# stanFurrer/Robust-Multimodal-Contrastive-Learning

Hardware: AMD Instinct MI355X
Metric: image-text pairs/sec, ViLT-B/32 RMCL step (PGD K=3) (higher is better)
Workload: dtype bf16; 1 GPU; RMCL step, PGD K=3 image attack + MoCo InfoNCE (queue 65536) + full backward + AdamW, ViLT-B/32, bs=64/GPU, 384x384 img + 40 tok (BASELINE configs[2]; [3] when n_gpus=8); global_batch=64, parallelism=dp1, grad_sync=ring/f32, ln_fold=on (shift-robust form)

## Files before the change

### robust-multimodal-contrastive-learning_amd/csrc/api.cpp

```cpp
#include "rmcl_common.h"
#include "kernels.h"
#include "../../include/rmcl.h"
#include <mutex>
#include <string>
#include <unordered_set>

static thread_local std::string g_err;
extern "C" void rmcl_set_error(const char* msg) { g_err = msg ? msg : ""; }

int rmcl_attention_fwd_impl(const void* qkv, const int* mask, void* out, void* probs, float* scores, int B, int N, int H, int dt,
                            int exact, hipStream_t s);
int rmcl_attention_bwd_impl(const void* qkv, const int* mask, const void* probs, const void* dout, const void* out, void* dqkv,
                            float* scores, void* dS, int B, int N, int H, int dt, int exact, hipStream_t s);

#include <vector>
namespace {
struct Prof {
  bool on = false;
  int mask = 0;
  size_t n = 0, cap = 0;
  std::vector<hipEvent_t> ev;
  double flops = 0.0;
} g_prof;
}
// ... 59 lines not shown
  g_prof.on = false;
  double ms = 0.0;
  for (size_t i = 0; i < g_prof.n; ++i) {
    hipError_t r = hipEventSynchronize(g_prof.ev[2 * i + 1]);
    float t = 0.f;
    if (r == hipSuccess) r = hipEventElapsedTime(&t, g_prof.ev[2 * i], g_prof.ev[2 * i + 1]);
    if (r != hipSuccess) { rmcl_set_error(hipGetErrorString(r)); return (int)r; }
    ms += t;
  }
  if (ms_total) *ms_total = ms;
  if (launches) *launches = (int64_t)g_prof.n;
  if (flops_total) *flops_total = g_prof.flops;
  return 0;
}
int rmcl_version(void) { return 1; }

int rmcl_dropout_mask_apply(float* x, int64_t n, uint32_t drop_seed, int layer, int site, float drop_p, void* stream) {
  RMCL_REQUIRE(x && drop_p >= 0.f && drop_p < 1.f, "dropout_mask_apply: bad argument");
  if (drop_p == 0.f) return 0;
  return rmcl_dropout_apply(x, n, rmcl_site_seed(drop_seed, layer, site), (uint32_t)((double)drop_p * 4294967296.0), 1.0f / (1.0f - drop_p),
                            (hipStream_t)stream);
}
extern int g_st_reserve_cus;
extern bool g_attn_fused_bwd;
extern bool g_dw_grouped;
extern int g_attn_fwd_waves;
extern int g_infonce_fold;
extern int g_dp_stagger;
extern int g_attn_bwd_persist;
extern int g_attn_bwd_tpw;
extern int g_gemm_share;
extern bool g_lnfold_centred;
extern int g_prefetch_mask, g_prefetch_wgs;
int rmcl_l2_prefetch_experiment(const void* A, int64_t lda_bytes, int M, int rows_per_tile, int tiles_per_xcd, int col_tiles, const void* B,
                                int64_t ldb_bytes, int nB, int nk, int tick, int lead, int per_xcd, int wgs, int* counter, int64_t* stamps, void* stream) {
  RMCL_REQUIRE(A && B && counter && M > 0 && nk > 0 && per_xcd > 0 && wgs > 0 && col_tiles > 0, "l2_prefetch_experiment: bad argument");
  return rmcl_debug_l2_prefetch(A, (long)lda_bytes, M, rows_per_tile, tiles_per_xcd, col_tiles, B, (long)ldb_bytes, nB, nk, tick, lead, per_xcd, wgs, counter,
                                reinterpret_cast<long long*>(stamps), (hipStream_t)stream);
}
int rmcl_tune_set(int key, int value) {
  if (key == 11) { g_lnfold_centred = value != 0; return 0; }
  if (key == 12) { g_prefetch_mask = value & 7; return 0; }
  if (key == 13) { g_prefetch_wgs = value < 0 ? 0 : (value > 64 ? 64 : value); return 0; }
  if (key == 7) { g_dp_stagger = value < 0 ? 0 : value; return 0; }
  if (key == 10) { g_gemm_share = value < 1 ? 1 : (value > 8 ? 8 : value); return 0; }
  if (key == 9) { g_attn_bwd_tpw = value; return 0; }
  if (key == 8) { g_attn_bwd_persist = value < 0 ? 0 : value; return 0; }
  if (key == 6) { rmcl_gemm_skinny_set_form(value); return 0; }
  if (key == 0) { rmcl_gemm_fast_set_cfg(value); return 0; }
  if (key == 1) { g_st_reserve_cus = value < 0 ? 0 : (value > 128 ? 128 : value); return 0; }
  if (key == 2) { g_attn_fused_bwd = value != 0; return 0; }
  if (key == 5) { g_infonce_fold = value != 0; return 0; }
  if (key == 4) { g_attn_fwd_waves = value; return 0; }
  if (key == 3) { g_dw_grouped = value != 0; return 0; }
  rmcl_set_error("tune_set: unknown key");
  return -1;
}

int64_t rmcl_heads_stash_bytes(const rmcl_dims* d) { return (int64_t)carve_heads(*d, nullptr, nullptr) + 256; }

int rmcl_heads_forward(const rmcl_dims* d, const float* pool32, const float* head32, const float* xn, void* hstash,
                       float* cls_feats, float* q, void* stream) {
  return rmcl_heads_forward2(d, pool32, head32, xn, hstash, cls_feats, q, 0, stream);
}
int rmcl_heads_forward2(const rmcl_dims* d, const float* pool32, const float* head32, const float* xn, void* hstash,
                        float* cls_feats, float* q, int flags, void* stream) {
  RMCL_REQUIRE(d && pool32 && xn && hstash && cls_feats, "heads_forward: NULL argument");
  RMCL_REQUIRE((flags & ~RMCL_HEADS_NO_WGRAD) == 0, "heads_forward: unknown flag");
  rmcl_layout y;
  rmcl_param_layout(d, &y);
  HeadStash h;
  carve_heads(*d, hstash, &h);
  hipStream_t s = (hipStream_t)stream;
  const int B = d->B, D = d->D, N = d->L + 1 + d->P;
  const bool stash_in = !(flags & RMCL_HEADS_NO_WGRAD);
  {
// ... 353 lines not shown
```

### robust-multimodal-contrastive-learning_amd/csrc/gemm_st.hip

```cpp
#include "rmcl_common.h"
#include "kernels.h"

#define ST_OP_BYTES (ST_T * 128)
#define ST_STAGE (2 * ST_OP_BYTES)
#define ST_LDS (3 * ST_STAGE)


#ifdef ST_TRACE
#ifndef ST_TRACE_WG
#define ST_TRACE_WG 100
#endif
__device__ long long g_st_trace[2][32];
#define ST_STAMP(i)                                                                                              \
  if (blockIdx.x == ST_TRACE_WG && (threadIdx.x & 255) == 0) g_st_trace[threadIdx.x >> 8][i] = wall_clock64()
extern "C" int rmcl_debug_st_trace(long long* out) {
  return (int)hipMemcpyFromSymbol(out, HIP_SYMBOL(g_st_trace), sizeof(long long) * 64);
}
__device__ long long g_dw_trace[2][32];
#define DW_STAMP(i)                                                                                              \
  if (blockIdx.x == ST_TRACE_WG && (threadIdx.x & 255) == 0) g_dw_trace[threadIdx.x >> 8][i] = wall_clock64()
extern "C" int rmcl_debug_dw_trace(long long* out) {
  return (int)hipMemcpyFromSymbol(out, HIP_SYMBOL(g_dw_trace), sizeof(long long) * 64);
}
#else
// ... 19 lines not shown
__device__ __forceinline__ bf16x8 st_ld_b(const char* lds_b, int off, int s) {
  if (KC) {
    return *reinterpret_cast<const bf16x8*>(lds_b + off);
  } else {
    union { bf16x8 v; s16x4 h[2]; } u;
    const uint32_t a = lds_addr(lds_b + off);
    if (s == 0) { u.h[0] = lds_read_tr16_asm<0>(a); u.h[1] = lds_read_tr16_asm<4 * 384>(a); }
    else { u.h[0] = lds_read_tr16_asm<32 * 384>(a); u.h[1] = lds_read_tr16_asm<32 * 384 + 4 * 384>(a); }
    return u.v;
  }
}

#define ST_PHASE_BEGIN()                                  \
  __builtin_amdgcn_sched_barrier(0);                      \
  __builtin_amdgcn_s_barrier();                           \
  asm volatile("s_waitcnt lgkmcnt(0)" ::: "memory");      \
  __builtin_amdgcn_sched_barrier(0);                      \
  __builtin_amdgcn_s_setprio(1)
#define ST_PHASE_END()                                    \
  __builtin_amdgcn_s_setprio(0);                          \
  __builtin_amdgcn_sched_barrier(0);                      \
  __builtin_amdgcn_s_barrier();                           \
  __builtin_amdgcn_sched_barrier(0)

struct STCtx {
  const bf16_t* A;
  const bf16_t* B;
  uint32_t oa[3], ob[3];
  int aoff[2], aoffi[6], boff[2], boffj[3];
  long kstep_a, kstep_b;
  int wave;
};

template <int MODE, bool A_KC, bool B_KC, int PH>
__device__ __forceinline__ void st_tile(f32x4 (&acc)[6][3], const STCtx& c, const char* cur, char* nxt2, int t2) {
  if constexpr (PH == 2) {
    bf16x8 a[6], b[3];
#pragma unroll
    for (int s = 0; s < 2; ++s) {
#pragma unroll
      for (int j = 0; j < 3; ++j) b[j] = B_KC ? st_ld_b<true>(cur + ST_OP_BYTES, j * 2048 + c.boff[s], s) : st_ld_b<false>(cur + ST_OP_BYTES, c.boffj[j], s);
#pragma unroll
      for (int i = 0; i < 6; ++i) a[i] = A_KC ? st_ld_b<true>(cur, i * 2048 + c.aoff[s], s) : st_ld_b<false>(cur, c.aoffi[i], s);
      if (MODE == 0) {
        if (s == 0) st_stage_op(c.A, c.oa, (long)t2 * c.kstep_a, nxt2, c.wave);
        else { st_stage_op(c.B, c.ob, (long)t2 * c.kstep_b, nxt2 + ST_OP_BYTES, c.wave); st_wait_vm<6>(); }
      } else if (MODE == 1 && s == 1) {
        st_wait_vm<0>();
      }
      asm volatile("s_waitcnt lgkmcnt(0)" ::: "memory");
      ST_PHASE_BEGIN();
#pragma unroll
      for (int i = 0; i < 6; ++i)
#pragma unroll
        for (int j = 0; j < 3; ++j) acc[i][j] = __builtin_amdgcn_mfma_f32_16x16x32_bf16(b[j], a[i], acc[i][j], 0, 0, 0);
      ST_PHASE_END();
    }
  } else {
    bf16x8 a[2][6], b[2][3];
#pragma unroll
    for (int s = 0; s < 2; ++s) {
#pragma unroll
      for (int j = 0; j < 3; ++j) b[s][j] = B_KC ? st_ld_b<true>(cur + ST_OP_BYTES, j * 2048 + c.boff[s], s) : st_ld_b<false>(cur + ST_OP_BYTES, c.boffj[j], s);
#pragma unroll
      for (int i = 0; i < 6; ++i) a[s][i] = A_KC ? st_ld_b<true>(cur, i * 2048 + c.aoff[s], s) : st_ld_b<false>(cur, c.aoffi[i], s);
    }
    if (MODE == 0) {
      st_stage_op(c.A, c.oa, (long)t2 * c.kstep_a, nxt2, c.wave);
      st_stage_op(c.B, c.ob, (long)t2 * c.kstep_b, nxt2 + ST_OP_BYTES, c.wave);
      st_wait_vm<6>();
    } else if (MODE == 1) {
      st_wait_vm<0>();
    }
    asm volatile("s_waitcnt lgkmcnt(0)" ::: "memory");
    ST_PHASE_BEGIN();
#pragma unroll
    for (int s = 0; s < 2; ++s)
#pragma unroll
      for (int i = 0; i < 6; ++i)
// ... 77 lines not shown
      float v[4] = {g.alpha * acc[i][j][0] + bias[j].x, g.alpha * acc[i][j][1] + bias[j].y, g.alpha * acc[i][j][2] + bias[j].z,
                    g.alpha * acc[i][j][3] + bias[j].w};
      if (DROP && (epi & EPI_DROP_BWD)) {
        const uint32_t di = (uint32_t)((long)m * g.ld_aux + nb + j * 16);
        drop_scale4(g.drop_seed, di, g.drop_thresh, g.drop_inv_keep, v[0], v[1], v[2], v[3]);
      }
      if (AUX == ST_AUX_DGELU) {
        const uint2 u = pre[i][j];
        v[0] *= gelu_poly_grad(__uint_as_float(u.x << 16)); v[1] *= gelu_poly_grad(__uint_as_float(u.x & 0xffff0000u));
        v[2] *= gelu_poly_grad(__uint_as_float(u.y << 16)); v[3] *= gelu_poly_grad(__uint_as_float(u.y & 0xffff0000u));
      }
      const long ci = (long)m * g.ldc + nb + j * 16;
      if ((epi & EPI_SAVE_PREACT) && live) st_store4<TO>(C2 + ci, v);
      if (epi & EPI_GELU) {
#pragma unroll
        for (int r = 0; r < 4; ++r) v[r] = gelu_poly(v[r]);
      }
      if (DROP && (epi & EPI_DROPOUT)) {
        drop_scale4(g.drop_seed, (uint32_t)ci, g.drop_thresh, g.drop_inv_keep, v[0], v[1], v[2], v[3]);
      }
      if (AUX == ST_AUX_RES) { v[0] += res[i][j].x; v[1] += res[i][j].y; v[2] += res[i][j].z; v[3] += res[i][j].w; }
      if constexpr (sizeof(TO) == 4) {
        if ((epi & EPI_ACCUM) && live) {
          const float4 o = *reinterpret_cast<const float4*>(C + ci);
          v[0] += o.x; v[1] += o.y; v[2] += o.z; v[3] += o.w;
        }
      }
      if (live) st_store4<TO>(C + ci, v);
    }
  }
}


template <bool A_KC, bool B_KC, int AUX, typename TO, bool DROP, int PH, int LNF = 0>
__global__ __launch_bounds__(512) void gemm_st_kernel(GemmArgs g, int tiles_m, int tiles_n, int rows_per_tile, int xflags) {
  extern __shared__ __attribute__((aligned(16))) char smem[];
  const int t = threadIdx.x, lane = t & 63;
  const int wave = __builtin_amdgcn_readfirstlane(t >> 6);
  const int wm = wave >> 2, wn = wave & 3;
  const int ntiles = tiles_m * tiles_n * max(g.splitk, 1), G = gridDim.x, bidx = blockIdx.x;

  STCtx c;
  c.A = reinterpret_cast<const bf16_t*>(g.A);
  c.B = reinterpret_cast<const bf16_t*>(g.B);
  c.wave = wave;
  c.kstep_a = A_KC ? 64 : 64 * g.lda;
  c.kstep_b = B_KC ? 64 : 64 * g.ldb;
#pragma unroll
  for (int i = 0; i < 6; ++i) {
    const int q = (lane & 15) >> 2, p = lane & 3;
    const int k = 8 * (lane >> 4) + q;
    const int c8 = (wm * 96 + i * 16) / 4 + p;
    c.aoffi[i] = k * 384 + (((c8 >> 1) ^ (st_gk(k) << 1)) * 16) + (c8 & 1) * 8;
  }
#pragma unroll
  for (int s = 0; s < 2; ++s) {
    const int sw = ((4 * s + (lane >> 4)) ^ (lane & 7)) * 16;
    c.aoff[s] = (wm * 96 + (lane & 15)) * 128 + sw;
    c.boff[s] = (wn * 48 + (lane & 15)) * 128 + sw;
  }
#pragma unroll
  for (int j = 0; j < 3; ++j) {
    const int q = (lane & 15) >> 2, p = lane & 3;
    const int k = 8 * (lane >> 4) + q;
    const int c8 = (wn * 48 + j * 16) / 4 + p;
    c.boffj[j] = k * 384 + (((c8 >> 1) ^ (st_gk(k) << 1)) * 16) + (c8 & 1) * 8;
  }

  ST_STAMP(0);
  int id = st_tile_id(bidx, 0, G, ntiles);
  if (id < 0) return;
  STTile cur, nxt;
  st_tile_setup<A_KC, B_KC>(cur, g, id, tiles_m, tiles_n, rows_per_tile, wave, lane, xflags);
#pragma unroll
  for (int q = 0; q < 3; ++q) { c.oa[q] = cur.oa[q]; c.ob[q] = cur.ob[q]; }

  st_stage_op(c.A, c.oa, (long)cur.kt0 * c.kstep_a, smem, wave);
  st_stage_op(c.B, c.ob, (long)cur.kt0 * c.kstep_b, smem + ST_OP_BYTES, wave);
  st_stage_op(c.A, c.oa, (long)(cur.kt0 + 1) * c.kstep_a, smem + ST_STAGE, wave);
  st_stage_op(c.B, c.ob, (long)(cur.kt0 + 1) * c.kstep_b, smem + ST_STAGE + ST_OP_BYTES, wave);
  st_wait_vm<6>();
  __builtin_amdgcn_s_barrier();
  __builtin_amdgcn_sched_barrier(0);
  if (wm == 1) __builtin_amdgcn_s_barrier();
  __builtin_amdgcn_sched_barrier(0);

  ST_STAMP(1);
  int sc = 0, sn = 2;
  for (int r = 0;; ++r) {
    const int nid = st_tile_id(bidx, r + 1, G, ntiles);
    f32x4 acc[6][3];
#pragma unroll
    for (int i = 0; i < 6; ++i)
#pragma unroll
      for (int j = 0; j < 3; ++j) acc[i][j] = f32x4{0.f, 0.f, 0.f, 0.f};
    const int nk = cur.nk;
    for (int it = 0; it + 2 < nk; ++it) {
      st_tile<0, A_KC, B_KC, PH>(acc, c, smem + sc * ST_STAGE, smem + sn * ST_STAGE, cur.kt0 + it + 2);
      sc = sc == 2 ? 0 : sc + 1;
      sn = sn == 2 ? 0 : sn + 1;
    }
    if (nid >= 0) {
      st_tile_setup<A_KC, B_KC>(nxt, g, nid, tiles_m, tiles_n, rows_per_tile, wave, lane, xflags);
#pragma unroll
      for (int q = 0; q < 3; ++q) { c.oa[q] = nxt.oa[q]; c.ob[q] = nxt.ob[q]; }
#pragma unroll
      for (int e = 0; e < 2; ++e) {
        st_tile<0, A_KC, B_KC, PH>(acc, c, smem + sc * ST_STAGE, smem + sn * ST_STAGE, nxt.kt0 + e);
        sc = sc == 2 ? 0 : sc + 1;
        sn = sn == 2 ? 0 : sn + 1;
      }
    } else {
      st_tile<1, A_KC, B_KC, PH>(acc, c, smem + sc * ST_STAGE, nullptr, 0);
      sc = sc == 2 ? 0 : sc + 1;
      st_tile<2, A_KC, B_KC, PH>(acc, c, smem + sc * ST_STAGE, nullptr, 0);
    }
    ST_STAMP(2);
    const int s_free = nid >= 0 ? (sc == 0 ? 2 : sc - 1) : sc;
    st_epilogue_lds<AUX, TO, DROP, LNF>(acc, g, cur, wm, wn, lane, wave, smem + s_free * ST_STAGE + wm * (ST_STAGE / 2),
                                        reinterpret_cast<float*>(smem + ST_LDS));
    if (nid < 0) break;
    cur = nxt;
  }
  ST_STAMP(20);
  if (wm == 0) __builtin_amdgcn_s_barrier();
#ifdef ST_TRACE
  asm volatile("s_waitcnt vmcnt(0)" ::: "memory");
  ST_STAMP(21);
#endif
}

__global__ __launch_bounds__(512) void gemm_dw_group_kernel(DwGroupArgs a) {
  extern __shared__ __attribute__((aligned(16))) char smem[];
  const int t = threadIdx.x, lane = t & 63;
  const int wave = __builtin_amdgcn_readfirstlane(t >> 6);
  const int wm = wave >> 2, wn = wave & 3;
  DW_STAMP(0);
  if ((int)blockIdx.x < a.nslots * ((a.D + 255) / 256) && t < 256) {
    const int per = (a.D + 255) / 256, si = blockIdx.x / per, c = (blockIdx.x % per) * 256 + t;
    if (c < a.D) {
      const float* base = a.rep + (long)a.slot[si] * (32 * 2 * 1024);
      float sg = 0.f, sb = 0.f;
#pragma unroll 8
      for (int r = 0; r < 32; ++r) { sg += base[r * 2048 + c]; sb += base[r * 2048 + 1024 + c]; }
      a.G[a.g_gamma[si] + c] += sg;
      a.G[a.g_beta[si] + c] += sb;
    }
  }
  const int ntiles = a.tile_base[4];
  const int id = st_tile_id(blockIdx.x, 0, gridDim.x, ntiles);
  if (id < 0) return;
  int gi = 0;
#pragma unroll
// ... 125 lines not shown
}

bool rmcl_gemm_st_supported(const GemmArgs& g, int a_kc, int b_kc) {
  if (g.nb1 > 1 || g.nb2 > 1) return false;
  if (g.N % ST_T != 0 || g.K % 64 != 0 || g.K < 128) return false;
  if ((long)(a_kc ? g.M : g.K) * g.lda >= (1L << 31) || (long)(b_kc ? g.N : g.K) * g.ldb >= (1L << 31)) return false;
  if (g.splitk > 1) return false;
  if ((long)g.M * g.ldc >= (1L << 31)) return false;
  if (!a_kc) {
    if (b_kc || g.M % ST_T != 0 || (g.epi & ~EPI_ACCUM)) return false;
    return true;
  }
  if (g.epi & ~(EPI_BIAS | EPI_GELU | EPI_SAVE_PREACT | EPI_RESIDUAL | EPI_DGELU | EPI_ACCUM | EPI_DROPOUT | EPI_DROP_BWD | EPI_LNFOLD | EPI_ROWSTAT)) return false;
  if ((g.epi & EPI_RESIDUAL) && (g.epi & EPI_DGELU)) return false;
  if (g.epi & EPI_LNFOLD) {
    if (!b_kc || (g.epi & ~(EPI_LNFOLD | EPI_GELU | EPI_SAVE_PREACT)) || ((g.epi & EPI_SAVE_PREACT) && !g.C2) || !g.ln_s || !g.ln_c || !g.ln_part ||
        g.ln_nparts % 2 || g.ln_nparts <= 0 || g.ln_cols <= 0)
      return false;
  }
  if (g.epi & EPI_ROWSTAT) {
    if (!b_kc || (g.epi & ~(EPI_ROWSTAT | EPI_BIAS | EPI_RESIDUAL | EPI_DROPOUT)) || !(g.epi & EPI_RESIDUAL) || !g.ln_part || !g.C2 || g.ln_nparts != 4 * (g.N / ST_T))
      return false;
  }
  return true;
}

double rmcl_gemm_st_fill(const GemmArgs& g, int cus) {
  const long tiles = (long)cdiv(g.M, ST_T) * (g.N / ST_T) * (g.splitk > 1 ? g.splitk : 1);
  return (double)tiles / (double)(cdiv(tiles, (long)cus) * cus);
}

int g_st_reserve_cus = 8;
int g_st_xflags = 0;

static int st_num_cus() {
  static int n = 0;
  if (!n) {
    int dev = 0;
    if (hipGetDevice(&dev) != hipSuccess || hipDeviceGetAttribute(&n, hipDeviceAttributeMultiprocessorCount, dev) != hipSuccess || n <= 0) n = 256;
  }
  return n;
}

template <bool A_KC, bool B_KC, int AUX, typename TO, bool DROP = false>
static int launch_st3(const GemmArgs& g, hipStream_t s) {
  static RmclLdsOnce once2, once1;
  RMCL_TRY(rmcl_set_max_lds(once2, reinterpret_cast<const void*>(gemm_st_kernel<A_KC, B_KC, AUX, TO, DROP, 2>), ST_LDS));
  RMCL_TRY(rmcl_set_max_lds(once1, reinterpret_cast<const void*>(gemm_st_kernel<A_KC, B_KC, AUX, TO, DROP, 1>), ST_LDS));
  const int tm = cdiv(g.M, ST_T), tn = g.N / ST_T, rows = A_KC ? cdiv(g.M, tm) : ST_T;
  const int items = tm * tn * (g.splitk > 1 ? g.splitk : 1);
  const int ncu = st_num_cus(), gres = max(8, ncu - (A_KC ? g_st_reserve_cus : 0));
  const int grid = min(items, cdiv(items, gres) > cdiv(items, ncu) ? ncu : gres);
  const bool one_phase = ((g_st_xflags & 4) != 0) != (!A_KC || !B_KC);
  if (one_phase) RMCL_LAUNCH((gemm_st_kernel<A_KC, B_KC, AUX, TO, DROP, 1>), dim3(grid), dim3(512), ST_LDS, s, g, tm, tn, rows, g_st_xflags);
  else RMCL_LAUNCH((gemm_st_kernel<A_KC, B_KC, AUX, TO, DROP, 2>), dim3(grid), dim3(512), ST_LDS, s, g, tm, tn, rows, g_st_xflags);
  RMCL_CHECK_LAUNCH();
  return 0;
}

template <bool B_KC, int AUX>
static int launch_st2(const GemmArgs& g, int dt_out, hipStream_t s) {
  if (g.epi & (EPI_DROPOUT | EPI_DROP_BWD))
    return dt_out == RMCL_F32 ? launch_st3<true, B_KC, AUX, float, true>(g, s) : launch_st3<true, B_KC, AUX, bf16_t, true>(g, s);
  return dt_out == RMCL_F32 ? launch_st3<true, B_KC, AUX, float>(g, s) : launch_st3<true, B_KC, AUX, bf16_t>(g, s);
}

template <bool B_KC>
static int launch_st(const GemmArgs& g, int dt_out, hipStream_t s) {
  if (g.epi & EPI_RESIDUAL) return launch_st2<B_KC, ST_AUX_RES>(g, dt_out, s);
  if (g.epi & EPI_DGELU) return launch_st2<B_KC, ST_AUX_DGELU>(g, dt_out, s);
  return launch_st2<B_KC, ST_AUX_NONE>(g, dt_out, s);
}

template <int AUX, typename TO, int LNF, bool DROP = false>
static int launch_st_lnf(const GemmArgs& g, hipStream_t s) {
  constexpr int LDS = ST_LDS + (LNF != 0 ? 2048 : 0);
  static RmclLdsOnce once;
  RMCL_TRY(rmcl_set_max_lds(once, reinterpret_cast<const void*>((gemm_st_kernel<true, true, AUX, TO, DROP, 2, LNF>)), LDS));
  const int tm = cdiv(g.M, ST_T), tn = g.N / ST_T, rows = cdiv(g.M, tm);
  const int grid = min(tm * tn, max(8, st_num_cus() - g_st_reserve_cus));
  RMCL_LAUNCH((gemm_st_kernel<true, true, AUX, TO, DROP, 2, LNF>), dim3(grid), dim3(512), LDS, s, g, tm, tn, rows, g_st_xflags);
  RMCL_CHECK_LAUNCH();
  return 0;
}

int rmcl_launch_gemm_st(const GemmArgs& g, int dt_out, int a_kc, int b_kc, hipStream_t s) {
  if (g.epi & EPI_LNFOLD) {
    RMCL_REQUIRE(a_kc && b_kc && dt_out == RMCL_BF16, "gemm_st: the LayerNorm-folded form is [rows][K] x [cols][K] with bf16 output");
    return launch_st_lnf<ST_AUX_NONE, bf16_t, 1>(g, s);
  }
  if (g.epi & EPI_ROWSTAT) {
    RMCL_REQUIRE(a_kc && b_kc && dt_out == RMCL_F32, "gemm_st: the row-statistics producer writes the fp32 residual stream");
    return (g.epi & EPI_DROPOUT) ? launch_st_lnf<ST_AUX_RES, float, 2, true>(g, s) : launch_st_lnf<ST_AUX_RES, float, 2>(g, s);
  }
  if (!a_kc) {
    RMCL_REQUIRE(dt_out == RMCL_F32 && !b_kc, "gemm_st: the [K][M] x [K][N] form writes fp32");
    return launch_st3<false, false, ST_AUX_NONE, float>(g, s);
  }
  return b_kc ? launch_st<true>(g, dt_out, s) : launch_st<false>(g, dt_out, s);
}

int rmcl_launch_gemm_st_slab(const GemmArgs& g0, float* slab, float* out, hipStream_t s) {
  GemmArgs g = g0;
  const int kts = g.K / 64;
  int sk = max(1, min(g.splitk, kts / 2));
  for (;; --sk) {
    const int per = cdiv(kts, sk), used = cdiv(kts, per);
    if (used == sk && kts - (sk - 1) * per >= 2) break;
    if (sk == 1) break;
  }
  g.splitk = sk;
  g.C = slab;
  g.ldc = g.N;
// ... 166 lines not shown
```

### robust-multimodal-contrastive-learning_amd/csrc/gemm_st_epi.h

```cpp
#pragma once
#include <type_traits>
#include "rmcl_common.h"
#include "kernels.h"

typedef __bf16 bf16x8 __attribute__((ext_vector_type(8)));
typedef __attribute__((address_space(3))) void lds_void;
typedef const __attribute__((address_space(1))) void glb_void;

#define ST_T 192
#ifndef ST_STAMP
#define ST_STAMP(i)
#endif

template <typename TO>
__device__ __forceinline__ void st_store4(TO* p, const float (&v)[4]) {
  if constexpr (sizeof(TO) == 2) {
    uint2 pk;
    pk.x = (uint32_t)f2bf(v[0]) | ((uint32_t)f2bf(v[1]) << 16);
    pk.y = (uint32_t)f2bf(v[2]) | ((uint32_t)f2bf(v[3]) << 16);
    *reinterpret_cast<uint2*>(p) = pk;
  } else {
    *reinterpret_cast<float4*>(p) = make_float4(v[0], v[1], v[2], v[3]);
  }
}

enum { ST_AUX_NONE = 0, ST_AUX_RES = 1, ST_AUX_DGELU = 2 };

struct STTile {
  uint32_t oa[3], ob[3];
  int m0, n0, m_end;
  int kt0, nk;
  long zoff;
};

__device__ __forceinline__ int st_tile_id(int b, int r, int G, int T) {
  const int n_r = min(G, T - r * G);
  if (n_r <= 0) return -1;
  const int x = b & 7, s = b >> 3, q = n_r >> 3, e = n_r & 7;
  if (s >= q + (x < e ? 1 : 0)) return -1;
  return r * G + (x < e ? x * (q + 1) : e * (q + 1) + (x - e) * q) + s;
}

template <int AUX, typename TO, bool DROP, int LNF = 0, bool ACCPRE = false>
__device__ __forceinline__ void st_epilogue_lds(const f32x4 (&acc)[6][3], const GemmArgs& g, const STTile& T, int wm, int wn, int lane, int wave,
                                                char* scratch, float* rowstat = nullptr) {
  constexpr int ESZ = sizeof(TO), RI = ESZ == 2 ? 3 : 2, NCH = 6 / RI, ROWS = RI * 16, ROWB = 192 * ESZ, PIECES = ROWB / 16;
  const int epi = g.epi;
  TO* C = reinterpret_cast<TO*>(g.C) + T.zoff;
  TO* C2 = reinterpret_cast<TO*>(g.C2);
  asm volatile("" : "+v"(lane));
  const int nb = T.n0 + wn * 48 + 4 * (lane >> 4);
  const int mb = T.m0 + wm * 96 + (lane & 15);
  float4 resb[2][AUX == ST_AUX_RES ? RI : 1][3];
  uint2 preb[2][AUX == ST_AUX_DGELU ? RI : 1][3];
  auto aux_fetch = [&](int ch, int buf) {
#pragma unroll
    for (int il = 0; il < RI; ++il) {
      const long mr = min(mb + (ch * RI + il) * 16, g.M - 1);
#pragma unroll
      for (int j = 0; j < 3; ++j) {
        if (AUX == ST_AUX_RES) resb[buf][il][j] = *reinterpret_cast<const float4*>(reinterpret_cast<const float*>(g.aux) + mr * g.ld_aux + nb + j * 16);
        if (AUX == ST_AUX_DGELU) preb[buf][il][j] = *reinterpret_cast<const uint2*>(reinterpret_cast<const bf16_t*>(g.aux) + mr * g.ld_aux + nb + j * 16);
      }
    }
  };
  if constexpr (AUX != ST_AUX_NONE) aux_fetch(0, 0);
  float4 bias[3], lns[LNF == 1 ? 3 : 1];
#pragma unroll
  for (int j = 0; j < 3; ++j) {
    if constexpr (LNF == 1) {
      bias[j] = *reinterpret_cast<const float4*>(g.ln_c + nb + j * 16);
      lns[j] = *reinterpret_cast<const float4*>(g.ln_s + nb + j * 16);
    } else {
      bias[j] = (epi & EPI_BIAS) ? *reinterpret_cast<const float4*>(g.bias + nb + j * 16) : make_float4(0.f, 0.f, 0.f, 0.f);
    }
  }
  if constexpr (LNF == 1) {
    const int tgs = (wave & 3) * 64 + lane;
    if (tgs < 96) {
      const int row = wm * 96 + tgs;
      const long m = min(T.m0 + row, g.M - 1);
      const float4* pp = reinterpret_cast<const float4*>(g.ln_part + m * (long)(g.ln_nparts * 2));
      const bool stash_m = T.n0 == 0 && g.ln_mean && T.m0 + row < T.m_end;
      const float cen = (stash_m && g.ln_center) ? g.ln_center[m] : 0.f;
      float s1 = 0.f, s2 = 0.f;
      if (g.ln_nparts == 16) {
        float4 v[8];
#pragma unroll
        for (int q = 0; q < 8; ++q) v[q] = pp[q];
#pragma unroll
        for (int q = 0; q < 8; ++q) { s1 += v[q].x + v[q].z; s2 += v[q].y + v[q].w; }
      } else {
        for (int q = 0; q < g.ln_nparts / 2; ++q) { const float4 v = pp[q]; s1 += v.x + v.z; s2 += v.y + v.w; }
      }
      const float inv = 1.0f / (float)g.ln_cols, mean = s1 * inv;
      const float rstd = rsqrtf(fmaxf(s2 * inv - mean * mean, 0.f) + g.ln_eps);
      rowstat[2 * row] = mean;
      rowstat[2 * row + 1] = rstd;
      if (stash_m) { g.ln_mean[m] = mean + cen; g.ln_rstd[m] = rstd; }
    }
    asm volatile("s_waitcnt lgkmcnt(0)" ::: "memory");
  }
  if constexpr (LNF == 2) {
    const int tgs = (wave & 3) * 64 + lane;
    if (tgs < 96) rowstat[wm * 96 + tgs] = g.ln_center ? g.ln_center[min(T.m0 + wm * 96 + tgs, g.M - 1)] : 0.f;
    asm volatile("s_waitcnt lgkmcnt(0)" ::: "memory");
  }
  ST_STAMP(3);
  __builtin_amdgcn_s_barrier();
  ST_STAMP(4);
  float2 rs[LNF == 1 ? 6 : 1];
  if constexpr (LNF == 1) {
#pragma unroll
    for (int i = 0; i < 6; ++i) rs[i] = *reinterpret_cast<const float2*>(rowstat + 2 * (wm * 96 + i * 16 + (lane & 15)));
  }
  float cen6[LNF == 2 ? 6 : 1];
  if constexpr (LNF == 2) {
#pragma unroll
    for (int i = 0; i < 6; ++i) cen6[i] = rowstat[wm * 96 + i * 16 + (lane & 15)];
  }
  constexpr int NIT = (ROWS * PIECES + 255) / 256;
  constexpr int RSTEP = 256 / PIECES, ROWS3 = 768 / PIECES, NT3 = (NIT + 2) / 3;
  int woff[3];
#pragma unroll
  for (int j = 0; j < 3; ++j) {
    const int r = lane & 15;
    if constexpr (ESZ == 2) {
      const int e8 = wn * 12 + j * 4 + (lane >> 4);
      woff[j] = r * ROWB + (((e8 >> 1) ^ (r & 7)) * 16) + (e8 & 1) * 8;
    } else {
      woff[j] = r * ROWB + (((wn * 12 + j * 4 + (lane >> 4)) ^ (r & 7)) * 16);
    }
  }
  int rb_row[3], rb_lds[3];
  uint32_t rb_dst[3];
  {
    const int tg = (wave & 3) * 64 + lane, row0 = tg / PIECES, cp0 = tg - row0 * PIECES;
#pragma unroll
    for (int kk = 0; kk < 3; ++kk) {
      const int t16 = cp0 + 16 * kk, wrap = (t16 >= PIECES ? 1 : 0) + (t16 >= 2 * PIECES ? 1 : 0), cp = t16 - wrap * PIECES;
      const int row = row0 + RSTEP * kk + wrap;
      rb_row[kk] = row;
      rb_lds[kk] = row * ROWB + cp * 16;
      rb_dst[kk] = (uint32_t)row * (uint32_t)g.ldc + (uint32_t)((cp ^ (row & 7)) * (16 / ESZ));
    }
  }
  float4 oldv[ACCPRE ? NCH : 1][ACCPRE ? NIT : 1];
  if constexpr (ACCPRE && ESZ == 4) {
#pragma unroll
    for (int ch = 0; ch < NCH; ++ch) {
      const int mrow = T.m0 + wm * 96 + ch * ROWS, lim = min(ROWS, T.m_end - mrow);
      const uint32_t cbase = (uint32_t)mrow * (uint32_t)g.ldc + (uint32_t)T.n0;
#pragma unroll
      for (int it = 0; it < NIT; ++it) {
        const int kk = it % 3, t3 = it / 3;
        oldv[ch][it] = make_float4(0.f, 0.f, 0.f, 0.f);
        if (rb_row[kk] + t3 * ROWS3 < lim)
          oldv[ch][it] = *reinterpret_cast<const float4*>(C + (size_t)(cbase + (uint32_t)(t3 * ROWS3) * (uint32_t)g.ldc + rb_dst[kk]));
      }
    }
  }
  const uint32_t dbase_aux = DROP ? (uint32_t)mb * (uint32_t)g.ld_aux + (uint32_t)nb : 0u, dbase_c = DROP ? (uint32_t)mb * (uint32_t)g.ldc + (uint32_t)nb : 0u;
  auto chunk_loop = [&](auto plain_c, auto dm_c) {
    constexpr bool PLAIN = decltype(plain_c)::value;
    constexpr int DM = decltype(dm_c)::value;
#pragma unroll
    for (int ch = 0; ch < NCH; ++ch) {
      if constexpr (AUX != ST_AUX_NONE) { if (ch + 1 < NCH) aux_fetch(ch + 1, (ch + 1) & 1); }
      auto& res = resb[ch & 1];
      auto& pre = preb[ch & 1];
#pragma unroll
      for (int il = 0; il < RI; ++il) {
        const int i = ch * RI + il;
        const int m = mb + i * 16;
        const bool live = m < T.m_end;
        float mean_m = 0.f, rstd_m = 1.f, ps1 = 0.f, ps2 = 0.f;
        if constexpr (LNF == 1) { mean_m = rs[i].x; rstd_m = rs[i].y; }
#pragma unroll
        for (int j = 0; j < 3; ++j) {
          const f32x4 av = acc[i][j], bv = f4v(bias[j]);
          f32x4 v;
          if constexpr (LNF == 1) v = rstd_m * (av - mean_m * f4v(lns[j])) + bv;
          else v = g.alpha * av + bv;
          if constexpr (DROP && (DM & 2) != 0) {
            if (DM == 2 || (epi & EPI_DROP_BWD)) {
              const uint32_t di = dbase_aux + (uint32_t)(i * 16) * (uint32_t)g.ld_aux + (uint32_t)(j * 16);
              drop_scale4(g.drop_seed, di, g.drop_thresh, g.drop_inv_keep, v);
            }
          }
          if (AUX == ST_AUX_DGELU) v *= gelu_poly_grad4(bf2f4(pre[il][j]));
          const long ci = (long)m * g.ldc + nb + j * 16;
          if (!PLAIN && (epi & EPI_SAVE_PREACT) && live) {
            const float t[4] = {v.x, v.y, v.z, v.w};
            st_store4<TO>(C2 + ci, t);
          }
          if (!PLAIN && (epi & EPI_GELU)) v = gelu_poly4(v);
          if constexpr (DROP && (DM & 1) != 0) {
            if (DM == 1 || (epi & EPI_DROPOUT))
              drop_scale4(g.drop_seed, dbase_c + (uint32_t)(i * 16) * (uint32_t)g.ldc + (uint32_t)(j * 16), g.drop_thresh, g.drop_inv_keep, v);
          }
          if (AUX == ST_AUX_RES) v += f4v(res[il][j]);
          if constexpr (LNF == 2) {
            const float c0 = cen6[i], d0 = v.x - c0, d1 = v.y - c0, d2 = v.z - c0, d3 = v.w - c0;
            ps1 += (d0 + d1) + (d2 + d3);
            ps2 += (d0 * d0 + d1 * d1) + (d2 * d2 + d3 * d3);
          }
          if constexpr (ESZ == 2) {
            *reinterpret_cast<uint2*>(scratch + woff[j] + il * 16 * ROWB) = f2bf4(v);
          } else {
            *reinterpret_cast<float4*>(scratch + woff[j] + il * 16 * ROWB) = make_float4(v.x, v.y, v.z, v.w);
          }
        }
        if constexpr (LNF == 2) {
          ps1 += __shfl_xor(ps1, 16, 64); ps1 += __shfl_xor(ps1, 32, 64);
          ps2 += __shfl_xor(ps2, 16, 64); ps2 += __shfl_xor(ps2, 32, 64);
          if (lane < 16 && live)
            *reinterpret_cast<float2*>(g.ln_part + ((long)m * g.ln_nparts + (T.n0 / ST_T) * 4 + wn) * 2) = make_float2(ps1, ps2);
        }
      }
      ST_STAMP(5 + 4 * ch);
      __builtin_amdgcn_s_barrier();
      ST_STAMP(6 + 4 * ch);
      {
        const int mrow = T.m0 + wm * 96 + ch * ROWS, lim = min(ROWS, T.m_end - mrow);
        const uint32_t cbase = (uint32_t)mrow * (uint32_t)g.ldc + (uint32_t)T.n0;
#pragma unroll
        for (int t3 = 0; t3 < NT3; ++t3)
#pragma unroll
          for (int kk = 0; kk < 3; ++kk) {
            if (kk + 3 * t3 < NIT && rb_row[kk] + t3 * ROWS3 < lim) {
              const float4 w = *reinterpret_cast<const float4*>(scratch + rb_lds[kk] + t3 * ROWS3 * ROWB);
              const size_t off = (size_t)(cbase + (uint32_t)(t3 * ROWS3) * (uint32_t)g.ldc + rb_dst[kk]);
              TO* dst = C + off;
              if constexpr (ESZ == 4) {
                float4 o = w;
                if constexpr (ACCPRE) {
                  const float4 old = oldv[ch][kk + 3 * t3];
                  o.x += old.x; o.y += old.y; o.z += old.z; o.w += old.w;
                } else if (!PLAIN && (epi & EPI_ACCUM)) {
                  const float4 old = *reinterpret_cast<const float4*>(dst);
                  o.x += old.x; o.y += old.y; o.z += old.z; o.w += old.w;
                }
                *reinterpret_cast<float4*>(dst) = o;
                if constexpr (LNF == 2) {
                  const float c0 = rowstat[wm * 96 + ch * ROWS + rb_row[kk] + t3 * ROWS3];
                  const uint2 pk = make_uint2(f2bf2(f32x2{o.x, o.y} - c0), f2bf2(f32x2{o.z, o.w} - c0));
                  *reinterpret_cast<uint2*>(reinterpret_cast<bf16_t*>(g.C2) + off) = pk;
                }
              } else {
                *reinterpret_cast<float4*>(dst) = w;
              }
            }
          }
      }
      ST_STAMP(7 + 4 * ch);
      __builtin_amdgcn_s_barrier();
      ST_STAMP(8 + 4 * ch);
    }
  };
  {
    using P0 = std::integral_constant<bool, false>;
    using P1 = std::integral_constant<bool, true>;
    const bool plain = !(epi & (EPI_GELU | EPI_SAVE_PREACT | EPI_ACCUM));
    if constexpr (!DROP) {
      if (plain) chunk_loop(P1{}, std::integral_constant<int, 0>{}); else chunk_loop(P0{}, std::integral_constant<int, 0>{});
    } else {
      const int dm = ((epi & EPI_DROPOUT) ? 1 : 0) | ((epi & EPI_DROP_BWD) ? 2 : 0);
      if (plain && dm == 1) chunk_loop(P1{}, std::integral_constant<int, 1>{});
      else if (plain && dm == 2) chunk_loop(P1{}, std::integral_constant<int, 2>{});
      else if (plain) chunk_loop(P1{}, std::integral_constant<int, 3>{});
      else chunk_loop(P0{}, std::integral_constant<int, 3>{});
    }
  }
  __builtin_amdgcn_s_barrier();
}
```

Baseline: 1945 pairs/s.

## Stage fp32 residual tiles into LDS during the last k-tiles of stream-K GEMM

Adds a residual-through-LDS variant of the stream-K GEMM for fp32 residual-add epilogues, used only when every tile gets its own workgroup. The residual tile is fetched straight into LDS with global_load_lds during the final two k-steps and the epilogue. Bias and LN centre values are parked in LDS at kernel start. This overlaps residual traffic with the MFMA tail and removes per-lane global residual loads from the epilogue critical path. In exchange it needs more LDS, a new template instantiation, and fine-grained waitcnt choreography that could hurt scheduling.

```diff
diff --git a/robust-multimodal-contrastive-learning_amd/csrc/api.cpp b/robust-multimodal-contrastive-learning_amd/csrc/api.cpp
--- a/robust-multimodal-contrastive-learning_amd/csrc/api.cpp
+++ b/robust-multimodal-contrastive-learning_amd/csrc/api.cpp
@@ -115,6 +115,7 @@
 extern int g_gemm_share;
 extern bool g_lnfold_centred;
 extern int g_prefetch_mask, g_prefetch_wgs;
+extern int g_st_res_lds;
 int rmcl_l2_prefetch_experiment(const void* A, int64_t lda_bytes, int M, int rows_per_tile, int tiles_per_xcd, int col_tiles, const void* B,
                                 int64_t ldb_bytes, int nB, int nk, int tick, int lead, int per_xcd, int wgs, int* counter, int64_t* stamps, void* stream) {
   RMCL_REQUIRE(A && B && counter && M > 0 && nk > 0 && per_xcd > 0 && wgs > 0 && col_tiles > 0, "l2_prefetch_experiment: bad argument");
@@ -125,6 +126,7 @@
   if (key == 11) { g_lnfold_centred = value != 0; return 0; }
   if (key == 12) { g_prefetch_mask = value & 7; return 0; }
   if (key == 13) { g_prefetch_wgs = value < 0 ? 0 : (value > 64 ? 64 : value); return 0; }
+  if (key == 14) { g_st_res_lds = value != 0; return 0; }
   if (key == 7) { g_dp_stagger = value < 0 ? 0 : value; return 0; }
   if (key == 10) { g_gemm_share = value < 1 ? 1 : (value > 8 ? 8 : value); return 0; }
   if (key == 9) { g_attn_bwd_tpw = value; return 0; }
diff --git a/robust-multimodal-contrastive-learning_amd/csrc/gemm_st.hip b/robust-multimodal-contrastive-learning_amd/csrc/gemm_st.hip
--- a/robust-multimodal-contrastive-learning_amd/csrc/gemm_st.hip
+++ b/robust-multimodal-contrastive-learning_amd/csrc/gemm_st.hip
@@ -75,8 +75,14 @@
   int wave;
 };
 
-template <int MODE, bool A_KC, bool B_KC, int PH>
-__device__ __forceinline__ void st_tile(f32x4 (&acc)[6][3], const STCtx& c, const char* cur, char* nxt2, int t2) {
+struct STRes {
+  const GemmArgs& g;
+  int m0, n0, lane;
+};
+
+template <int MODE, bool A_KC, bool B_KC, int PH, bool RES = false>
+__device__ __forceinline__ void st_tile(f32x4 (&acc)[6][3], const STCtx& c, const char* cur, char* nxt2, int t2, const STRes* rx = nullptr) {
+  static_assert(!RES || (PH == 2 && MODE != 0), "residual staging: the last two k-tiles of the two-phase form");
   if constexpr (PH == 2) {
     bf16x8 a[6], b[3];
 #pragma unroll
@@ -88,6 +94,10 @@
       if (MODE == 0) {
         if (s == 0) st_stage_op(c.A, c.oa, (long)t2 * c.kstep_a, nxt2, c.wave);
         else { st_stage_op(c.B, c.ob, (long)t2 * c.kstep_b, nxt2 + ST_OP_BYTES, c.wave); st_wait_vm<6>(); }
+      } else if constexpr (RES) {
+#pragma unroll
+        for (int q = 0; q < 3; ++q) st_stage_res(rx->g, rx->m0, rx->n0, MODE - 1, s * 3 + q, nxt2, c.wave, rx->lane);
+        if (MODE == 1 && s == 1) st_wait_vm<6>();
       } else if (MODE == 1 && s == 1) {
         st_wait_vm<0>();
       }
@@ -231,7 +241,7 @@
 }
 
 
-template <bool A_KC, bool B_KC, int AUX, typename TO, bool DROP, int PH, int LNF = 0>
+template <bool A_KC, bool B_KC, int AUX, typename TO, bool DROP, int PH, int LNF = 0, bool RESL = false>
 __global__ __launch_bounds__(512) void gemm_st_kernel(GemmArgs g, int tiles_m, int tiles_n, int rows_per_tile, int xflags) {
   extern __shared__ __attribute__((aligned(16))) char smem[];
   const int t = threadIdx.x, lane = t & 63;
@@ -274,6 +284,17 @@
 #pragma unroll
   for (int q = 0; q < 3; ++q) { c.oa[q] = cur.oa[q]; c.ob[q] = cur.ob[q]; }
 
+  if constexpr (RESL) {
+    float* park = reinterpret_cast<float*>(smem + ST_LDS);
+    if (LNF == 2 && wave < 3) {
+      if (g.ln_center) __builtin_amdgcn_global_load_lds((glb_void*)(g.ln_center + min(cur.m0 + wave * 64 + lane, g.M - 1)), (lds_void*)(park + wave * 64), 4, 0, 0);
+      else park[wave * 64 + lane] = 0.f;
+    } else if (wave >= 4 && wave < 7) {
+      if (g.epi & EPI_BIAS) __builtin_amdgcn_global_load_lds((glb_void*)(g.bias + cur.n0 + (wave - 4) * 64 + lane), (lds_void*)(park + ST_RES_BIAS + (wave - 4) * 64), 4, 0, 0);
+      else park[ST_RES_BIAS + (wave - 4) * 64 + lane] = 0.f;
+    }
+    asm volatile("s_waitcnt lgkmcnt(0)" ::: "memory");
+  }
   st_stage_op(c.A, c.oa, (long)cur.kt0 * c.kstep_a, smem, wave);
   st_stage_op(c.B, c.ob, (long)cur.kt0 * c.kstep_b, smem + ST_OP_BYTES, wave);
   st_stage_op(c.A, c.oa, (long)(cur.kt0 + 1) * c.kstep_a, smem + ST_STAGE, wave);
@@ -287,7 +308,7 @@
   ST_STAMP(1);
   int sc = 0, sn = 2;
   for (int r = 0;; ++r) {
-    const int nid = st_tile_id(bidx, r + 1, G, ntiles);
+    const int nid = RESL ? -1 : st_tile_id(bidx, r + 1, G, ntiles);
     f32x4 acc[6][3];
 #pragma unroll
     for (int i = 0; i < 6; ++i)
@@ -309,6 +330,14 @@
         sc = sc == 2 ? 0 : sc + 1;
         sn = sn == 2 ? 0 : sn + 1;
       }
+    } else if constexpr (RESL) {
+      int rl = lane;
+      asm volatile("" : "+v"(rl));
+      const STRes rx{g, cur.m0, cur.n0, rl};
+      const int s1 = sc;
+      st_tile<1, A_KC, B_KC, PH, true>(acc, c, smem + sc * ST_STAGE, smem + sn * ST_STAGE, 0, &rx);
+      sc = sc == 2 ? 0 : sc + 1;
+      st_tile<2, A_KC, B_KC, PH, true>(acc, c, smem + sc * ST_STAGE, smem + s1 * ST_STAGE, 0, &rx);
     } else {
       st_tile<1, A_KC, B_KC, PH>(acc, c, smem + sc * ST_STAGE, nullptr, 0);
       sc = sc == 2 ? 0 : sc + 1;
@@ -316,8 +345,8 @@
     }
     ST_STAMP(2);
     const int s_free = nid >= 0 ? (sc == 0 ? 2 : sc - 1) : sc;
-    st_epilogue_lds<AUX, TO, DROP, LNF>(acc, g, cur, wm, wn, lane, wave, smem + s_free * ST_STAGE + wm * (ST_STAGE / 2),
-                                        reinterpret_cast<float*>(smem + ST_LDS));
+    st_epilogue_lds<AUX, TO, DROP, LNF, false, RESL>(acc, g, cur, wm, wn, lane, wave, smem + s_free * ST_STAGE + wm * (ST_STAGE / 2),
+                                                     reinterpret_cast<float*>(smem + ST_LDS), s_free);
     if (nid < 0) break;
     cur = nxt;
   }
@@ -509,6 +538,11 @@
 
 int g_st_reserve_cus = 8;
 int g_st_xflags = 0;
+int g_st_res_lds = 1;
+
+static bool st_res_lds_ok(const GemmArgs& g, int items, int grid) {
+  return g_st_res_lds != 0 && items <= grid && g.aux && g.splitk <= 1 && !(g.epi & (EPI_GELU | EPI_SAVE_PREACT | EPI_ACCUM));
+}
 
 static int st_num_cus() {
   static int n = 0;
@@ -529,6 +563,15 @@
   const int ncu = st_num_cus(), gres = max(8, ncu - (A_KC ? g_st_reserve_cus : 0));
   const int grid = min(items, cdiv(items, gres) > cdiv(items, ncu) ? ncu : gres);
   const bool one_phase = ((g_st_xflags & 4) != 0) != (!A_KC || !B_KC);
+  if constexpr (A_KC && B_KC && AUX == ST_AUX_RES && sizeof(TO) == 4) {
+    if (!one_phase && st_res_lds_ok(g, items, grid)) {
+      static RmclLdsOnce once_r;
+      RMCL_TRY(rmcl_set_max_lds(once_r, reinterpret_cast<const void*>(gemm_st_kernel<true, true, AUX, TO, DROP, 2, 0, true>), ST_LDS + 2048));
+      RMCL_LAUNCH((gemm_st_kernel<true, true, AUX, TO, DROP, 2, 0, true>), dim3(grid), dim3(512), ST_LDS + 2048, s, g, tm, tn, rows, g_st_xflags);
+      RMCL_CHECK_LAUNCH();
+      return 0;
+    }
+  }
   if (one_phase) RMCL_LAUNCH((gemm_st_kernel<A_KC, B_KC, AUX, TO, DROP, 1>), dim3(grid), dim3(512), ST_LDS, s, g, tm, tn, rows, g_st_xflags);
   else RMCL_LAUNCH((gemm_st_kernel<A_KC, B_KC, AUX, TO, DROP, 2>), dim3(grid), dim3(512), ST_LDS, s, g, tm, tn, rows, g_st_xflags);
   RMCL_CHECK_LAUNCH();
@@ -556,6 +599,15 @@
   RMCL_TRY(rmcl_set_max_lds(once, reinterpret_cast<const void*>((gemm_st_kernel<true, true, AUX, TO, DROP, 2, LNF>)), LDS));
   const int tm = cdiv(g.M, ST_T), tn = g.N / ST_T, rows = cdiv(g.M, tm);
   const int grid = min(tm * tn, max(8, st_num_cus() - g_st_reserve_cus));
+  if constexpr (LNF == 2 && AUX == ST_AUX_RES && sizeof(TO) == 4) {
+    if (st_res_lds_ok(g, tm * tn, grid)) {
+      static RmclLdsOnce once_r;
+      RMCL_TRY(rmcl_set_max_lds(once_r, reinterpret_cast<const void*>((gemm_st_kernel<true, true, AUX, TO, DROP, 2, LNF, true>)), LDS));
+      RMCL_LAUNCH((gemm_st_kernel<true, true, AUX, TO, DROP, 2, LNF, true>), dim3(grid), dim3(512), LDS, s, g, tm, tn, rows, g_st_xflags);
+      RMCL_CHECK_LAUNCH();
+      return 0;
+    }
+  }
   RMCL_LAUNCH((gemm_st_kernel<true, true, AUX, TO, DROP, 2, LNF>), dim3(grid), dim3(512), LDS, s, g, tm, tn, rows, g_st_xflags);
   RMCL_CHECK_LAUNCH();
   return 0;
diff --git a/robust-multimodal-contrastive-learning_amd/csrc/gemm_st_epi.h b/robust-multimodal-contrastive-learning_amd/csrc/gemm_st_epi.h
--- a/robust-multimodal-contrastive-learning_amd/csrc/gemm_st_epi.h
+++ b/robust-multimodal-contrastive-learning_amd/csrc/gemm_st_epi.h
@@ -41,9 +41,45 @@
   return r * G + (x < e ? x * (q + 1) : e * (q + 1) + (x - e) * q) + s;
 }
 
-template <int AUX, typename TO, bool DROP, int LNF = 0, bool ACCPRE = false>
+#define ST_STAGE_BYTES (2 * ST_T * 128)
+#define ST_RES_BIAS 256
+__device__ __forceinline__ void st_stage_res(const GemmArgs& g, int m0, int n0, int ch, int q, char* stage, int wave, int lane) {
+  const int wm = wave >> 2, pw = (wave & 3) * 6 + q;
+  const int L = pw * 1024 + lane * 16, r = L / 768, p = (L - r * 768) >> 4;
+  const long m = min(m0 + wm * 96 + ch * 32 + r, g.M - 1);
+  const float* src = reinterpret_cast<const float*>(g.aux) + m * g.ld_aux + n0 + ((p ^ (r & 7)) << 2);
+  __builtin_amdgcn_global_load_lds((glb_void*)src, (lds_void*)(stage + wm * (ST_STAGE_BYTES / 2) + pw * 1024), 16, 0, 0);
+}
+
+__device__ __forceinline__ f32x4 st_lds_read128(uint32_t a) {
+  f32x4 v;
+  asm volatile("ds_read_b128 %0, %1" : "=v"(v) : "v"(a) : "memory");
+  return v;
+}
+__device__ __forceinline__ float st_lds_read32(uint32_t a) {
+  float v;
+  asm volatile("ds_read_b32 %0, %1" : "=v"(v) : "v"(a) : "memory");
+  return v;
+}
+__device__ __forceinline__ void st_lds_write128(uint32_t a, f32x4 v) {
+  asm volatile("ds_write_b128 %0, %1" : : "v"(a), "v"(v) : "memory");
+}
+__device__ __forceinline__ void st_lds_wait(f32x4 (&a)[6]) {
+  asm volatile("s_waitcnt lgkmcnt(0)" : "+v"(a[0]), "+v"(a[1]), "+v"(a[2]), "+v"(a[3]), "+v"(a[4]), "+v"(a[5]) : : "memory");
+}
+__device__ __forceinline__ void st_lds_wait(f32x4 (&a)[3], float (&b)[6]) {
+  asm volatile("s_waitcnt lgkmcnt(0)" : "+v"(a[0]), "+v"(a[1]), "+v"(a[2]), "+v"(b[0]), "+v"(b[1]), "+v"(b[2]), "+v"(b[3]), "+v"(b[4]), "+v"(b[5]) : : "memory");
+}
+__device__ __forceinline__ void st_lds_wait(f32x4 (&a)[6], float (&b)[6]) {
+  asm volatile("s_waitcnt lgkmcnt(0)"
+               : "+v"(a[0]), "+v"(a[1]), "+v"(a[2]), "+v"(a[3]), "+v"(a[4]), "+v"(a[5]), "+v"(b[0]), "+v"(b[1]), "+v"(b[2]), "+v"(b[3]), "+v"(b[4]), "+v"(b[5])
+               : : "memory");
+}
+
+template <int AUX, typename TO, bool DROP, int LNF = 0, bool ACCPRE = false, bool RESL = false>
 __device__ __forceinline__ void st_epilogue_lds(const f32x4 (&acc)[6][3], const GemmArgs& g, const STTile& T, int wm, int wn, int lane, int wave,
-                                                char* scratch, float* rowstat = nullptr) {
+                                                char* scratch, float* rowstat = nullptr, int sc = 0) {
+  static_assert(!RESL || (AUX == ST_AUX_RES && sizeof(TO) == 4 && LNF != 1 && !ACCPRE), "residual through LDS: fp32 residual producers");
   constexpr int ESZ = sizeof(TO), RI = ESZ == 2 ? 3 : 2, NCH = 6 / RI, ROWS = RI * 16, ROWB = 192 * ESZ, PIECES = ROWB / 16;
   const int epi = g.epi;
   TO* C = reinterpret_cast<TO*>(g.C) + T.zoff;
@@ -51,7 +87,7 @@
   asm volatile("" : "+v"(lane));
   const int nb = T.n0 + wn * 48 + 4 * (lane >> 4);
   const int mb = T.m0 + wm * 96 + (lane & 15);
-  float4 resb[2][AUX == ST_AUX_RES ? RI : 1][3];
+  float4 resb[2][AUX == ST_AUX_RES && !RESL ? RI : 1][3];
   uint2 preb[2][AUX == ST_AUX_DGELU ? RI : 1][3];
   auto aux_fetch = [&](int ch, int buf) {
 #pragma unroll
@@ -64,13 +100,19 @@
       }
     }
   };
-  if constexpr (AUX != ST_AUX_NONE) aux_fetch(0, 0);
+  if constexpr (AUX != ST_AUX_NONE && !RESL) aux_fetch(0, 0);
+  auto img = [&](int ch) -> char* {
+    if constexpr (!RESL) return scratch;
+    const int d = sc + 1 + ch;
+    return scratch + ((d >= 3 ? d - 3 : d) - sc) * ST_STAGE_BYTES;
+  };
   float4 bias[3], lns[LNF == 1 ? 3 : 1];
 #pragma unroll
   for (int j = 0; j < 3; ++j) {
     if constexpr (LNF == 1) {
       bias[j] = *reinterpret_cast<const float4*>(g.ln_c + nb + j * 16);
       lns[j] = *reinterpret_cast<const float4*>(g.ln_s + nb + j * 16);
+    } else if constexpr (RESL) {
     } else {
       bias[j] = (epi & EPI_BIAS) ? *reinterpret_cast<const float4*>(g.bias + nb + j * 16) : make_float4(0.f, 0.f, 0.f, 0.f);
     }
@@ -101,21 +143,43 @@
     }
     asm volatile("s_waitcnt lgkmcnt(0)" ::: "memory");
   }
-  if constexpr (LNF == 2) {
+  if constexpr (LNF == 2 && !RESL) {
     const int tgs = (wave & 3) * 64 + lane;
     if (tgs < 96) rowstat[wm * 96 + tgs] = g.ln_center ? g.ln_center[min(T.m0 + wm * 96 + tgs, g.M - 1)] : 0.f;
     asm volatile("s_waitcnt lgkmcnt(0)" ::: "memory");
   }
+  float cen6[LNF == 2 ? 6 : 1];
+  if constexpr (RESL) {
+    static_assert(RI == 2, "residual through LDS: six 16-byte units per lane and chunk");
+    f32x4 bq[3];
+    float cq[6];
+    const uint32_t ba = lds_addr(rowstat + ST_RES_BIAS + wn * 48 + 4 * (lane >> 4)), ca = lds_addr(rowstat + wm * 96 + (lane & 15));
+#pragma unroll
+    for (int j = 0; j < 3; ++j) bq[j] = st_lds_read128(ba + j * 64);
+#pragma unroll
+    for (int i = 0; i < 6; ++i) cq[i] = LNF == 2 ? st_lds_read32(ca + i * 64) : 0.f;
+    st_lds_wait(bq, cq);
+#pragma unroll
+    for (int j = 0; j < 3; ++j) bias[j] = make_float4(bq[j][0], bq[j][1], bq[j][2], bq[j][3]);
+    if constexpr (LNF == 2) {
+#pragma unroll
+      for (int i = 0; i < 6; ++i) cen6[i] = cq[i];
+    }
+  }
   ST_STAMP(3);
+  if constexpr (RESL) asm volatile("s_waitcnt vmcnt(6)" ::: "memory");
   __builtin_amdgcn_s_barrier();
   ST_STAMP(4);
+  if constexpr (RESL) {
+#pragma unroll
+    for (int q = 0; q < 6; ++q) st_stage_res(g, T.m0, T.n0, 2, q, scratch - wm * (ST_STAGE_BYTES / 2), wave, lane);
+  }
   float2 rs[LNF == 1 ? 6 : 1];
   if constexpr (LNF == 1) {
 #pragma unroll
     for (int i = 0; i < 6; ++i) rs[i] = *reinterpret_cast<const float2*>(rowstat + 2 * (wm * 96 + i * 16 + (lane & 15)));
   }
-  float cen6[LNF == 2 ? 6 : 1];
-  if constexpr (LNF == 2) {
+  if constexpr (LNF == 2 && !RESL) {
 #pragma unroll
     for (int i = 0; i < 6; ++i) cen6[i] = rowstat[wm * 96 + i * 16 + (lane & 15)];
   }
@@ -166,9 +230,20 @@
     constexpr int DM = decltype(dm_c)::value;
 #pragma unroll
     for (int ch = 0; ch < NCH; ++ch) {
-      if constexpr (AUX != ST_AUX_NONE) { if (ch + 1 < NCH) aux_fetch(ch + 1, (ch + 1) & 1); }
-      auto& res = resb[ch & 1];
+      if constexpr (AUX != ST_AUX_NONE && !RESL) { if (ch + 1 < NCH) aux_fetch(ch + 1, (ch + 1) & 1); }
+      auto& res = resb[RESL ? 0 : ch & 1];
       auto& pre = preb[ch & 1];
+      char* const scr = img(ch);
+      float2 psd[RESL && LNF == 2 ? RI : 1];
+      f32x4 rr[RESL ? 6 : 1];
+      if constexpr (RESL) {
+        const uint32_t sa = lds_addr(scr);
+#pragma unroll
+        for (int il = 0; il < RI; ++il)
+#pragma unroll
+          for (int j = 0; j < 3; ++j) rr[il * 3 + j] = st_lds_read128(sa + woff[j] + il * 16 * ROWB);
+        st_lds_wait(rr);
+      }
 #pragma unroll
       for (int il = 0; il < RI; ++il) {
         const int i = ch * RI + il;
@@ -199,23 +274,40 @@
             if (DM == 1 || (epi & EPI_DROPOUT))
               drop_scale4(g.drop_seed, dbase_c + (uint32_t)(i * 16) * (uint32_t)g.ldc + (uint32_t)(j * 16), g.drop_thresh, g.drop_inv_keep, v);
           }
-          if (AUX == ST_AUX_RES) v += f4v(res[il][j]);
+          if constexpr (RESL) v += rr[il * 3 + j];
+          else if (AUX == ST_AUX_RES) v += f4v(res[il][j]);
           if constexpr (LNF == 2) {
             const float c0 = cen6[i], d0 = v.x - c0, d1 = v.y - c0, d2 = v.z - c0, d3 = v.w - c0;
             ps1 += (d0 + d1) + (d2 + d3);
             ps2 += (d0 * d0 + d1 * d1) + (d2 * d2 + d3 * d3);
           }
           if constexpr (ESZ == 2) {
-            *reinterpret_cast<uint2*>(scratch + woff[j] + il * 16 * ROWB) = f2bf4(v);
+            *reinterpret_cast<uint2*>(scr + woff[j] + il * 16 * ROWB) = f2bf4(v);
+          } else if constexpr (RESL) {
+            st_lds_write128(lds_addr(scr) + woff[j] + il * 16 * ROWB, v);
           } else {
-            *reinterpret_cast<float4*>(scratch + woff[j] + il * 16 * ROWB) = make_float4(v.x, v.y, v.z, v.w);
+            *reinterpret_cast<float4*>(scr + woff[j] + il * 16 * ROWB) = make_float4(v.x, v.y, v.z, v.w);
           }
         }
         if constexpr (LNF == 2) {
           ps1 += __shfl_xor(ps1, 16, 64); ps1 += __shfl_xor(ps1, 32, 64);
           ps2 += __shfl_xor(ps2, 16, 64); ps2 += __shfl_xor(ps2, 32, 64);
-          if (lane < 16 && live)
+          if constexpr (RESL) psd[il] = make_float2(ps1, ps2);
+          else if (lane < 16 && live)
             *reinterpret_cast<float2*>(g.ln_part + ((long)m * g.ln_nparts + (T.n0 / ST_T) * 4 + wn) * 2) = make_float2(ps1, ps2);
+        }
+      }
+      if constexpr (RESL) {
+        asm volatile("s_waitcnt lgkmcnt(0)" ::: "memory");
+        if (ch == 0) asm volatile("s_waitcnt vmcnt(6)" ::: "memory");
+        else if (ch == 1) asm volatile("s_waitcnt vmcnt(0)" ::: "memory");
+        if constexpr (LNF == 2) {
+#pragma unroll
+          for (int il = 0; il < RI; ++il) {
+            const int m = mb + (ch * RI + il) * 16;
+            if (lane < 16 && m < T.m_end)
+              *reinterpret_cast<float2*>(g.ln_part + ((long)m * g.ln_nparts + (T.n0 / ST_T) * 4 + wn) * 2) = psd[il];
+          }
         }
       }
       ST_STAMP(5 + 4 * ch);
@@ -224,12 +316,28 @@
       {
         const int mrow = T.m0 + wm * 96 + ch * ROWS, lim = min(ROWS, T.m_end - mrow);
         const uint32_t cbase = (uint32_t)mrow * (uint32_t)g.ldc + (uint32_t)T.n0;
+        f32x4 wq[RESL ? 6 : 1];
+        float cq[RESL ? 6 : 1];
+        if constexpr (RESL) {
+          static_assert(NIT == 6 && NT3 == 2, "residual through LDS: six read-back units per lane and chunk");
+          const uint32_t sa = lds_addr(scr), ca = lds_addr(rowstat + wm * 96 + ch * ROWS);
+#pragma unroll
+          for (int t3 = 0; t3 < NT3; ++t3)
+#pragma unroll
+            for (int kk = 0; kk < 3; ++kk) {
+              wq[kk + 3 * t3] = st_lds_read128(sa + rb_lds[kk] + t3 * ROWS3 * ROWB);
+              cq[kk + 3 * t3] = LNF == 2 ? st_lds_read32(ca + 4 * (rb_row[kk] + t3 * ROWS3)) : 0.f;
+            }
+          st_lds_wait(wq, cq);
+        }
 #pragma unroll
         for (int t3 = 0; t3 < NT3; ++t3)
 #pragma unroll
           for (int kk = 0; kk < 3; ++kk) {
             if (kk + 3 * t3 < NIT && rb_row[kk] + t3 * ROWS3 < lim) {
-              const float4 w = *reinterpret_cast<const float4*>(scratch + rb_lds[kk] + t3 * ROWS3 * ROWB);
+              float4 w;
+              if constexpr (RESL) { const f32x4 u = wq[kk + 3 * t3]; w = make_float4(u[0], u[1], u[2], u[3]); }
+              else w = *reinterpret_cast<const float4*>(scr + rb_lds[kk] + t3 * ROWS3 * ROWB);
               const size_t off = (size_t)(cbase + (uint32_t)(t3 * ROWS3) * (uint32_t)g.ldc + rb_dst[kk]);
               TO* dst = C + off;
               if constexpr (ESZ == 4) {
@@ -243,7 +351,7 @@
                 }
                 *reinterpret_cast<float4*>(dst) = o;
                 if constexpr (LNF == 2) {
-                  const float c0 = rowstat[wm * 96 + ch * ROWS + rb_row[kk] + t3 * ROWS3];
+                  const float c0 = RESL ? cq[RESL ? kk + 3 * t3 : 0] : rowstat[wm * 96 + ch * ROWS + rb_row[kk] + t3 * ROWS3];
                   const uint2 pk = make_uint2(f2bf2(f32x2{o.x, o.y} - c0), f2bf2(f32x2{o.z, o.w} - c0));
                   *reinterpret_cast<uint2*>(reinterpret_cast<bf16_t*>(g.C2) + off) = pk;
                 }
@@ -262,13 +370,15 @@
     using P0 = std::integral_constant<bool, false>;
     using P1 = std::integral_constant<bool, true>;
     const bool plain = !(epi & (EPI_GELU | EPI_SAVE_PREACT | EPI_ACCUM));
-    if constexpr (!DROP) {
+    if constexpr (RESL && !DROP) {
+      chunk_loop(P1{}, std::integral_constant<int, 0>{});
+    } else if constexpr (!DROP) {
       if (plain) chunk_loop(P1{}, std::integral_constant<int, 0>{}); else chunk_loop(P0{}, std::integral_constant<int, 0>{});
     } else {
       const int dm = ((epi & EPI_DROPOUT) ? 1 : 0) | ((epi & EPI_DROP_BWD) ? 2 : 0);
       if (plain && dm == 1) chunk_loop(P1{}, std::integral_constant<int, 1>{});
       else if (plain && dm == 2) chunk_loop(P1{}, std::integral_constant<int, 2>{});
-      else if (plain) chunk_loop(P1{}, std::integral_constant<int, 3>{});
+      else if (plain || RESL) chunk_loop(P1{}, std::integral_constant<int, 3>{});
       else chunk_loop(P0{}, std::integral_constant<int, 3>{});
     }
   }
```

Result: faster. 1969 pairs/s (median of 6 runs) (+1.2%).
